# kspalaiologos/bzip3

Hardware: AMD Instinct MI355X
Metric: MiB/s encode+decode round-trip, 8 MiB blocks (higher is better)
Workload: dtype u8

## Files before the change

### bzip3_amd/__init__.py

```python
import ctypes as C
import os

_HERE = os.path.dirname(os.path.abspath(__file__))
LIB_PATH = os.path.join(_HERE, "lib", "libbzip3.so")

BZ3_OK = 0
BZ3_ERR_OUT_OF_BOUNDS = -1
BZ3_ERR_BWT = -2
BZ3_ERR_CRC = -3
BZ3_ERR_MALFORMED_HEADER = -4
BZ3_ERR_TRUNCATED_DATA = -5
BZ3_ERR_DATA_TOO_BIG = -6
BZ3_ERR_INIT = -7
BZ3_ERR_DATA_SIZE_TOO_SMALL = -8

T_NAMES = ["crc", "rle", "lzp", "bwt", "cm", "copy", "_6", "_7"]

_lib = None


def _declare(L, strict=True):
    vp, i32, u32, sz = C.c_void_p, C.c_int32, C.c_uint32, C.c_size_t
    sig = {
        "bz3_version": (C.c_char_p, []),
        "bz3_last_error": (C.c_int8, [vp]),
        "bz3_strerror": (C.c_char_p, [vp]),
        "bz3_new": (vp, [i32]),
        "bz3_free": (None, [vp]),
        "bz3_bound": (sz, [sz]),
        "bz3_compress": (C.c_int, [u32, vp, vp, sz, C.POINTER(sz)]),
        "bz3_decompress": (C.c_int, [vp, vp, sz, C.POINTER(sz)]),
        "bz3_min_memory_needed": (sz, [i32]),
        "bz3_encode_block": (i32, [vp, vp, i32]),
        "bz3_decode_block": (i32, [vp, vp, sz, i32, i32]),
        "bz3_encode_blocks": (None, [vp, vp, vp, i32]),
        "bz3_decode_blocks": (None, [vp, vp, vp, vp, vp, i32]),
        "bz3_orig_size_sufficient_for_decode": (C.c_int, [vp, sz, i32]),
        "bz3_hip_device_count": (C.c_int, []),
        "bz3_hip_bind_device": (C.c_int, [C.c_int]),
        "bz3_hip_state_device": (C.c_int, [vp]),
        "bz3_hip_set_cm_mode": (C.c_int, [C.c_int]),
        "bz3_hip_cm_blocks_given_up": (C.c_uint, []),
        "bz3_hip_cm_blocks_routed_full": (C.c_uint, []),
        "bz3_hip_debug_bwt_big_rounds": (None, [C.c_int]),
        "bz3_hip_debug_peak_concurrent_groups": (C.c_int, [C.c_int]),
        "bz3_hip_debug_front_end_ring": (C.c_int, []),
        "bz3_hip_debug_arena_swap_buffers": (C.c_int, [C.c_int]),
        "bz3_hip_cm_variant_for": (C.c_int, [C.c_int, C.c_int, C.c_int]),
        "bz3_hip_set_lean_states": (C.c_int, [C.c_int]),
        "bz3_hip_release_cached_memory": (None, []),
        "bz3_hip_set_keep_workspace": (C.c_int, [C.c_int]),
        "bz3_hip_set_front_end_duo": (C.c_int, [C.c_int]),
        "bz3_hip_set_workspace_headroom": (None, [C.c_longlong]),
        "bz3_hip_workspace_headroom": (sz, []),
        "bz3_hip_debug_headroom_events": (C.c_uint, [C.c_int, C.POINTER(C.c_uint)]),
        "bz3_hip_debug_ring_contexts": (sz, [sz, sz, sz, sz, sz, sz, C.c_int, sz]),
        "bz3_hip_debug_arena_slack": (sz, [sz]),
        "bz3_hip_debug_cm_launches": (C.c_uint, [C.c_int]),
        "bz3_hip_debug_workspace_bytes": (sz, [sz, C.c_int]),
        "bz3_hip_debug_cached_bytes": (sz, [C.c_int]),
        "bz3_hip_encode_block_device": (i32, [vp, vp, i32]),
        "bz3_hip_decode_block_device": (i32, [vp, vp, sz, i32, i32]),
        "bz3_hip_encode_blocks_device": (None, [vp, vp, vp, i32]),
        "bz3_hip_decode_blocks_device": (None, [vp, vp, vp, vp, vp, i32]),
        "bz3_hip_compress_device": (C.c_int, [u32, vp, vp, sz, C.POINTER(sz)]),
        "bz3_hip_decompress_device": (C.c_int, [vp, vp, sz, C.POINTER(sz)]),
        "bz3_hip_frame_decoded_size_device": (C.c_int, [vp, sz, C.POINTER(sz)]),
        "bz3_hip_compress_device_many": (C.c_int, [u32, i32, C.POINTER(vp), C.POINTER(sz), C.POINTER(vp), C.POINTER(sz), C.POINTER(C.c_int)]),
        "bz3_hip_decompress_device_many": (C.c_int, [i32, C.POINTER(vp), C.POINTER(sz), C.POINTER(vp), C.POINTER(sz), C.POINTER(C.c_int)]),
        "bz3_hip_frame_decoded_sizes_device": (C.c_int, [i32, C.POINTER(vp), C.POINTER(sz), C.POINTER(sz), C.POINTER(C.c_int)]),
        "bz3_hip_debug_copy_segments": (i32, [vp, vp, C.POINTER(C.c_uint64), i32]),
        "bz3_hip_compress_device_planes": (C.c_int, [u32, u32, vp, vp, sz, C.POINTER(sz)]),
        "bz3_hip_decompress_device_planes": (C.c_int, [u32, vp, vp, sz, C.POINTER(sz)]),
        "bz3_hip_compress_device_planes_many": (C.c_int, [u32, i32, C.POINTER(u32), C.POINTER(vp), C.POINTER(sz), C.POINTER(vp), C.POINTER(sz), C.POINTER(C.c_int)]),
        "bz3_hip_decompress_device_planes_many": (C.c_int, [i32, C.POINTER(u32), C.POINTER(vp), C.POINTER(sz), C.POINTER(vp), C.POINTER(sz), C.POINTER(C.c_int)]),
        "bz3_hip_debug_planes": (i32, [vp, vp, C.POINTER(C.c_uint64), i32]),
        "bz3_hip_compress_device_delta": (C.c_int, [u32, u32, vp, vp, vp, sz, C.POINTER(sz)]),
        "bz3_hip_decompress_device_delta": (C.c_int, [u32, vp, vp, sz, vp, sz, C.POINTER(sz)]),
        "bz3_hip_compress_device_delta_many": (C.c_int, [u32, i32, C.POINTER(u32), C.POINTER(vp), C.POINTER(vp), C.POINTER(sz), C.POINTER(vp), C.POINTER(sz), C.POINTER(C.c_int)]),
        "bz3_hip_decompress_device_delta_many": (C.c_int, [i32, C.POINTER(u32), C.POINTER(vp), C.POINTER(sz), C.POINTER(vp), C.POINTER(sz), C.POINTER(vp), C.POINTER(sz), C.POINTER(C.c_int)]),
        "bz3_hip_crc32c_device": (C.c_int, [vp, sz, u32, C.POINTER(u32)]),
        "bz3_hip_debug_delta": (i32, [vp, vp, vp, C.POINTER(C.c_uint64), i32]),
        "bz3_hip_decompress_device_range": (C.c_int, [u32, vp, sz, C.c_uint64, vp, sz, vp, C.POINTER(sz)]),
        "bz3_hip_decompress_device_range_many": (C.c_int, [i32, C.POINTER(u32), C.POINTER(vp), C.POINTER(sz), C.POINTER(C.c_uint64), C.POINTER(vp), C.POINTER(sz),
                                                           C.POINTER(vp), C.POINTER(sz), C.POINTER(C.c_int)]),
# ... 705 lines not shown
```

### bzip3_amd/csrc/api.hip

```cpp
#include <atomic>
#include <chrono>
#include <condition_variable>
#include <cstdio>
#include <cstdlib>
#include <exception>
#include <mutex>
#include <new>
#include <stdexcept>
#include <thread>
#include <type_traits>
#include <vector>

#include "../../include/bz3_hip.h"
#include "frame.hpp"
#include "planes.hpp"
#include "prims.hpp"
#include "sort.hpp"
#include "stages.hpp"

using namespace bz3;

namespace {

constexpr s32 KiB65 = 65 * 1024;
// ... 79 lines not shown
#endif
            for (int k = 0; k < AUX; k++) {
                HIP_CHECK(hipStreamCreateWithFlags(&st[k], hipStreamNonBlocking));
                HIP_CHECK(hipEventCreate(&e0[k]));
                HIP_CHECK(hipEventCreate(&e1[k]));
            }
            HIP_CHECK(hipStreamCreateWithFlags(&du, hipStreamNonBlocking));
        } catch (...) {
            if (du) (void)hipStreamDestroy(du);
            if (ep) (void)hipEventDestroy(ep);
            if (rs) (void)hipStreamDestroy(rs);
            for (int k = 0; k < AUX; k++)
                if (sm[k]) (void)hipStreamDestroy(sm[k]);
            for (int k = 0; k < AUX; k++) {
                if (st[k]) (void)hipStreamDestroy(st[k]);
                if (e0[k]) (void)hipEventDestroy(e0[k]);
                if (e1[k]) (void)hipEventDestroy(e1[k]);
            }
            throw;
        }
        ev_prep = ep;
        duo = du;
        rest = rs;
        for (int k = 0; k < AUX; k++) aux_m[k] = sm[k];
        reserved_cus = reserved;
        for (int k = 0; k < AUX; k++) {
            aux[k] = st[k];
            ev_d0[k] = e0[k];
            ev_d1[k] = e1[k];
        }
        aux_ready = true;
    }

    std::mutex temp_mu;
    std::vector<std::pair<u8 *, size_t>> temps_free;
    std::vector<std::pair<u8 *, size_t>> temps_out;
    u8 * temp_get(size_t cap) {
        std::lock_guard<std::mutex> lk(temp_mu);
        for (size_t k = 0; k < temps_free.size(); k++)
            if (temps_free[k].second >= cap) {
                auto t = temps_free[k];
                temps_free.erase(temps_free.begin() + (long)k);
                temps_out.push_back(t);
                return t.first;
            }
        u8 * p = nullptr;
        if (hipMalloc((void **)&p, cap) != hipSuccess) {
            (void)hipGetLastError();
            (void)hipDeviceSynchronize();
            for (auto & t : temps_free) (void)hipFree(t.first);
            temps_free.clear();
            HIP_CHECK(hipMalloc((void **)&p, cap));
        }
        temps_out.push_back({p, cap});
        return p;
    }
    void temp_put(u8 * p) {
        if (!p) return;
        std::lock_guard<std::mutex> lk(temp_mu);
        for (size_t k = 0; k < temps_out.size(); k++)
            if (temps_out[k].first == p) {
                temps_free.push_back(temps_out[k]);
                temps_out.erase(temps_out.begin() + (long)k);
                return;
            }
    }
// ... 368 lines not shown
    if (total <= base || !ctx_bytes) return 0;
    size_t by_share = (total - base) / 10 * 7 / ctx_bytes;
    const size_t aside = headroom + ((size_t)513 << 20) + ((size_t)64 << 20);
    const size_t room = total > base + aside ? total - base - aside : 0;
    if (!lean) {
        const size_t by_room = room / ctx_bytes;
        return by_share < by_room ? by_share : by_room;
    }
    return room / (ctx_bytes + cap);
}
void enforce_headroom(DeviceCtx * ctx, hipStream_t s);

#ifndef BZ3_FRONT_DUO_DEFAULT
#define BZ3_FRONT_DUO_DEFAULT 0
#endif
std::atomic<int> g_keep_ws{-1};
inline bool keep_workspace() {
    static const bool env_on = [] {
        const char * e = getenv("BZ3_HIP_KEEP_WS");
        return e && atoi(e) != 0;
    }();
    const int v = g_keep_ws.load();
    return v < 0 ? env_on : v != 0;
}
std::atomic<int> g_front_duo{-1};
inline bool front_end_duo() {
    static const int env_on = [] {
        const char * e = getenv("BZ3_HIP_FRONT_DUO");
        return e ? (atoi(e) != 0 ? 1 : 0) : BZ3_FRONT_DUO_DEFAULT;
    }();
    const int v = g_front_duo.load();
    return v < 0 ? env_on != 0 : v != 0;
}
inline void lean_borrow(bz3_state * st) {
    if (st->lean && !st->d_swap) st->d_swap = st->ctx->temp_get(st->cap);
}
inline void lean_return(bz3_state * st) {
    if (st->lean && st->d_swap) {
        st->ctx->temp_put(st->d_swap);
        st->d_swap = nullptr;
    }
}
constexpr u32 CM_SIDE_BYTES = 64 * 1024;

void encode_front_a(bz3_state * st, u8 * buf, s32 data_size, Arena & arena, Arena & ctx_arena, LzpEncodeCtx & c) {
    st->pending = bz3_state::FAILED;
    st->result = -1;
    c.active = false;
    if (st->skip) return;
    if (data_size > st->block_size || data_size < 0) {
        st->last_error = BZ3_ERR_DATA_TOO_BIG;
        return;
    }
    hipStream_t s = st->xs;
    for (float & x : st->t) x = 0.f;
    double t0 = now_ms();
    crc32c_device(buf, (u64)data_size, 1u, st->ctx->d_crc, st->d_words, s);
    st->user = buf;
    st->size = data_size;
    if (data_size < 64) {
        launch(k_store_small, dim3(1), dim3(64), 0, s, buf, (u32)data_size, (const u32 *)(st->d_words + 1));
        st->pending = bz3_state::ENC_STORED;
        return;
    }
    if (st->timed) {
        HIP_CHECK(hipStreamSynchronize(s));
// ... 143 lines not shown
    if (const char * e = getenv("BZ3_HIP_LZP_PIPE")) {
        int w = 0, q = 0;
        if (sscanf(e, "%d,%d", &w, &q) == 2 && w >= 1 && q >= 2 && q <= DeviceCtx::AUX) {
            window = w;
            ns = q;
        }
    }
    if (window > n) window = n;
    if (window < 1) window = 1;
}

void encode_group(bz3_state ** sts, u8 ** bufs, const s32 * sizes, s32 n) {
    if (n <= 0) return;
    bz3_state * lead = sts[0];
    DeviceGuard g(lead->device);
    std::lock_guard<std::mutex> lk(lead->ctx->mu);
    for (s32 i = 0; i < n; i++) {
        sts[i]->xs = lead->stream;
        sts[i]->timed = i == 0;
    }
    size_t need = 0, need_a = 0, need_b = 0;
    for (s32 i = 0; i < n; i++) {
        const u64 nb = (u64)(sizes[i] > 0 ? sizes[i] : 0) + 64;
        const size_t w = workspace_bytes_for(nb), wa = front_a_scratch_bytes(nb), wb = front_b_scratch_bytes(nb);
        if (w > need) need = w;
        if (wa > need_a) need_a = wa;
        if (wb > need_b) need_b = wb;
    }
    const bool duo_wanted = front_end_duo() && n >= 16;
    if (duo_wanted) need = need_a + need_b + 65536;
    u64 n_max = 64;
    for (s32 i = 0; i < n; i++)
        if (sizes[i] > 0 && (u64)sizes[i] > n_max) n_max = (u64)sizes[i];
    const size_t ctx_bytes = lzp_encode_ctx_bytes(n_max + 64) + 65536;
    const size_t headroom = ws_headroom();
    const size_t fixed = (size_t)n * (sizeof(CmEncodeJob) + CM_SIDE_BYTES + 256) + cm_scratch_bytes((size_t)n) + 65536 + (size_t)DeviceCtx::AUX * 8 * (sizeof(LzpDriverJob) + 256);
    size_t contexts = ((size_t)32 << 30) / ctx_bytes;
    {
        size_t free_b = 0, total_b = 0;
        const s32 full = DeviceCtx::RING_SLOTS * 8;
        if (lead->lean && lead->ctx->temp_idle_bytes() > 0 && hipMemGetInfo(&free_b, &total_b) == hipSuccess) {
            if (ring_contexts_for(free_b, lead->ctx->ws_cap, need, fixed, ctx_bytes, lead->cap, true, headroom) < (size_t)(n < full ? n : full)) lead->ctx->temp_trim();
        }
        if (hipMemGetInfo(&free_b, &total_b) == hipSuccess)
            contexts = ring_contexts_for(free_b, lead->ctx->ws_cap, need, fixed, ctx_bytes, lead->cap, lead->lean, headroom);
    }
    s32 window = 1, ns = 2;
    pipeline_shape((s32)(contexts < 1024 ? contexts : 1024), n, window, ns);
    lead->ctx->ensure_aux();
    hipStream_t s = lead->stream;
    DrainOnUnwind drain{s, lead->ctx->aux, DeviceCtx::AUX};
    static const bool front_rest = [] { const char * e = getenv("BZ3_HIP_FRONT_REST"); return e && atoi(e) != 0; }();
    if (front_rest && lead->ctx->rest && n > 1) {
        s = lead->ctx->rest;
        for (s32 i = 0; i < n; i++) sts[i]->xs = s;
    }
    DrainOnUnwind drain_rest{s == lead->stream ? nullptr : s, nullptr, 0};
    Arena arena;
    for (;;) {
        try {
            arena = lead->ctx->arena_for(need + (size_t)ns * (size_t)window * (ctx_bytes + sizeof(LzpDriverJob) + 256) +
                                         (size_t)n * (sizeof(CmEncodeJob) + CM_SIDE_BYTES + 256) + cm_scratch_bytes((size_t)n) + 65536);
            break;
        } catch (const HipError &) {
            if (ns == 2 && window == 1) throw;
            (void)hipGetLastError();
            if (ns > 2) ns = 2;
            else window = (window + 1) / 2;
        }
    }
    g_front_end_ring.store(window | (ns << 16));
    CmEncodeJob * d_jobs = arena.take<CmEncodeJob>((size_t)n);
    u8 * sides = arena.take<u8>((size_t)n * CM_SIDE_BYTES);
    struct Window {
        s32 w0 = 0, w1 = 0;
        Arena slot;
        LzpDriverJob * d_lz = nullptr;
        std::vector<LzpEncodeCtx> ctxs;
        std::vector<LzpDriverJob> lz;
    } win[DeviceCtx::AUX];
    for (int k = 0; k < ns; k++) {
        win[k].slot.base = arena.take<char>((size_t)window * ctx_bytes);
        win[k].slot.cap = (size_t)window * ctx_bytes;
        win[k].d_lz = arena.take<LzpDriverJob>((size_t)window);
    }
    std::vector<CmEncodeJob> jobs;
    std::vector<s32> job_owner;
    const s32 nwin = (n + window - 1) / window;
    const s32 lag = ns - 1;
    static const bool trace_rings = getenv("BZ3_HIP_TRACE_RINGS") != nullptr;
    double tr_prep = 0, tr_wait = 0, tr_fin = 0, tr_t0 = now_ms();
    auto prepare = [&](s32 k, hipStream_t sp, Arena & scr, hipEvent_t ev) {
        const int q = (int)(k % ns);
        Window & w = win[q];
        w.w0 = k * window;
        w.w1 = (w.w0 + window < n) ? w.w0 + window : n;
        w.slot.used = 0;
        w.ctxs.assign((size_t)(w.w1 - w.w0), LzpEncodeCtx());
        w.lz.clear();
        for (s32 i = w.w0; i < w.w1; i++) {
            sts[i]->xs = sp;
            sts[i]->hold_swap = false;
            encode_front_a(sts[i], bufs[i], sizes[i], scr, w.slot, w.ctxs[(size_t)(i - w.w0)]);
            if (sts[i]->pending == bz3_state::ENC_CODED && w.ctxs[(size_t)(i - w.w0)].active) w.lz.push_back(lzp_driver_job(w.ctxs[(size_t)(i - w.w0)]));
        }
        HIP_CHECK(hipEventRecord(ev, sp));
        if (!w.lz.empty()) {
            hipStream_t sq = lead->ctx->aux[q];
            HIP_CHECK(hipStreamWaitEvent(sq, ev, 0));
            HIP_CHECK(hipEventRecord(lead->ctx->ev_d0[q], sq));
            lzp_driver_batch(w.lz.data(), w.d_lz, (u32)w.lz.size(), sq);
            HIP_CHECK(hipEventRecord(lead->ctx->ev_d1[q], sq));
        }
    };
    auto finish = [&](s32 j, hipStream_t sf, Arena & scr, std::vector<bz3_state *> * held) {
        const int q = (int)(j % ns);
        Window & w = win[q];
        float driver_ms = 0.f;
        if (!w.lz.empty()) {
            const double t0 = now_ms();
            HIP_CHECK(hipEventSynchronize(lead->ctx->ev_d1[q]));
            (void)hipEventElapsedTime(&driver_ms, lead->ctx->ev_d0[q], lead->ctx->ev_d1[q]);
            tr_wait += now_ms() - t0;
        }
        for (s32 i = w.w0; i < w.w1; i++) {
            sts[i]->xs = sf;
            sts[i]->hold_swap = held != nullptr;
            encode_front_b(sts[i], scr, w.ctxs[(size_t)(i - w.w0)], driver_ms);
            sts[i]->hold_swap = false;
            if (sts[i]->pending == bz3_state::ENC_CODED) {
                CmEncodeJob j2{dev_addr(sts[i]->b2), dev_addr(sts[i]->b1 + sts[i]->overhead * 4 + 1), dev_addr(sts[i]->d_words + 2), sts[i]->n_cm, 0u};
                if (sts[i]->lean) {
                    sts[i]->side = sides + (size_t)i * CM_SIDE_BYTES;
                    j2.gap = (u32)(sts[i]->b2 - (sts[i]->b1 + sts[i]->overhead * 4 + 1));
                    j2.side = dev_addr(sts[i]->side);
                    j2.side_cap = CM_SIDE_BYTES;
                }
                jobs.push_back(j2);
                job_owner.push_back(i);
            }
            if (held) {
                if (sts[i]->lean && sts[i]->d_swap) held->push_back(sts[i]);
            } else {
                lean_return(sts[i]);
            }
        }
    };
    const bool duo = duo_wanted && nwin >= 3 && lead->ctx->aux_ready && s == lead->stream;
    if (!duo) {
        for (s32 k = 0; k < nwin + lag; k++) {
            const double tr_a = now_ms();
            if (k < nwin) prepare(k, s, arena, lead->ctx->ev_prep);
            const double tr_b = now_ms();
            tr_prep += tr_b - tr_a;
            if (k >= lag) finish(k - lag, s, arena, nullptr);
            tr_fin += now_ms() - tr_b;
        }
    } else {
        g_front_end_ring.fetch_or(1 << 29);
        hipStream_t sA = lead->ctx->duo;
        DrainOnUnwind drain_duo{sA, nullptr, 0};
        Arena scr_a;
        scr_a.base = arena.take<char>(need_a);
        scr_a.cap = need_a;
        struct Events {
            std::vector<hipEvent_t> e;
            ~Events() {
                for (hipEvent_t x : e)
                    if (x) (void)hipEventDestroy(x);
            }
        } evs;
        evs.e.assign((size_t)2 * (size_t)nwin, nullptr);
        for (auto & x : evs.e) HIP_CHECK(hipEventCreateWithFlags(&x, hipEventDisableTiming));
        hipEvent_t * evA = evs.e.data(), * evB = evs.e.data() + nwin;
        struct Shared {
            std::mutex m;
            std::condition_variable cv;
            s32 prepared = 0, finished = 0;
            bool abort = false;
            std::exception_ptr err;
            std::mutex pool;
            hipEvent_t last_return = nullptr;
// ... 52 lines not shown
            }
        } joiner{ta, sh};
        std::vector<bz3_state *> held;
        for (s32 j = 0; j < nwin; j++) {
            const double tr_b = now_ms();
            {
                std::unique_lock<std::mutex> ul(sh.m);
                sh.cv.wait(ul, [&] { return sh.abort || sh.prepared >= j + 1; });
                if (sh.abort) break;
            }
            HIP_CHECK(hipStreamWaitEvent(s, evA[j], 0));
            held.clear();
            finish(j, s, arena, &held);
            HIP_CHECK(hipEventRecord(evB[j], s));
            {
                std::lock_guard<std::mutex> pl(sh.pool);
                for (bz3_state * st : held) lean_return(st);
                sh.last_return = evB[j];
            }
            {
                std::lock_guard<std::mutex> ul(sh.m);
                sh.finished = j + 1;
            }
            sh.cv.notify_all();
            tr_fin += now_ms() - tr_b;
        }
        ta.join();
        if (sh.err) std::rethrow_exception(sh.err);
        HIP_CHECK(hipStreamSynchronize(sA));
        tr_prep = sh.prep_ms;
        for (s32 i = 0; i < n; i++) sts[i]->xs = s;
    }
    if (trace_rings)
        fprintf(stderr, "[bz3 rings] encode front end: %d blocks, %d windows of %d x %d slots: %.1f ms = CRC / mRLE / LZP prepare %.1f + waiting for a window's LZP drivers %.1f + LZP emit / BWT / header %.1f\n",
                (int)n, (int)nwin, (int)window, (int)ns, now_ms() - tr_t0, tr_prep, tr_wait, tr_fin - tr_wait);
    if (s != lead->stream) {
        HIP_CHECK(hipStreamSynchronize(s));
        s = lead->stream;
        for (s32 i = 0; i < n; i++) sts[i]->xs = s;
    }
    std::vector<char> to_full(jobs.size(), 0);
    if (jobs.size() > (size_t)lead->ctx->cus) {
        std::vector<u32> outside(jobs.size(), 0u);
        for (size_t k = 0; k < jobs.size(); k++) HIP_CHECK(hipMemcpyAsync(&outside[k], sts[job_owner[k]]->d_words + 8, 4, hipMemcpyDeviceToHost, lead->stream));
        HIP_CHECK(hipStreamSynchronize(lead->stream));
        for (size_t k = 0; k < jobs.size(); k++) to_full[k] = outside[k] > jobs[k].n / 4u ? 1 : 0;
    }
    const float cm_ms = run_cm_jobs(lead->ctx, arena, jobs, d_jobs, lead->stream, lead->ev0, lead->ev1,
                                    [](const CmEncodeJob * j, u32 nj, hipStream_t st, int variant) { cm_encode_batch(j, nj, st, variant); }, &to_full);
    for (s32 i = 0; i < n; i++) encode_finish(sts[i], cm_ms);
    size_t slack = (size_t)16 << 30;
    if (const char * e = getenv("BZ3_HIP_WS_KEEP_MB")) slack = (size_t)strtoull(e, nullptr, 10) << 20;
    if (lead->ctx->ws_cap > 2 * need + slack && !(keep_workspace() && lead->lean)) {
        HIP_CHECK(hipStreamSynchronize(s));
        (void)hipFree(lead->ctx->ws);
        lead->ctx->ws = nullptr;
        lead->ctx->ws_cap = 0;
        g_front_end_ring.fetch_or(1 << 30);
    }
    enforce_headroom(lead->ctx, lead->stream);
}

void decode_front(bz3_state * st, u8 * buf, size_t buffer_size, s32 compressed_size, s32 orig_size, const u8 * hdr) {
    st->pending = bz3_state::FAILED;
    st->result = -1;
    if (st->skip) return;
    if (buffer_size < 9 || buffer_size < (size_t)compressed_size) {
        st->last_error = BZ3_ERR_DATA_SIZE_TOO_SMALL;
// ... 717 lines not shown
}

BZIP3_API unsigned bz3_hip_cm_blocks_routed_full(void) { return g_cm_routed_full.load(); }
BZIP3_API void bz3_hip_set_workspace_headroom(long long bytes) { g_ws_headroom.store(bytes < 0 ? -1 : bytes); }
BZIP3_API size_t bz3_hip_workspace_headroom(void) { return ws_headroom(); }
BZIP3_API unsigned bz3_hip_debug_headroom_events(int reset, unsigned * releases) {
    const unsigned t = reset ? g_headroom_trims.exchange(0) : g_headroom_trims.load();
    const unsigned r = reset ? g_headroom_releases.exchange(0) : g_headroom_releases.load();
    if (releases) *releases = r;
    return t;
}
BZIP3_API size_t bz3_hip_debug_ring_contexts(size_t free_b, size_t have, size_t need, size_t fixed, size_t ctx_bytes, size_t cap, int lean, size_t headroom) {
    return ring_contexts_for(free_b, have, need, fixed, ctx_bytes, cap, lean != 0, headroom);
}
BZIP3_API size_t bz3_hip_debug_workspace_bytes(size_t block_bytes, int which) {
    return which == 0 ? workspace_bytes_for((u64)block_bytes + 64) : lzp_encode_ctx_bytes((u64)block_bytes + 64) + 65536;
}
BZIP3_API unsigned bz3_hip_debug_cm_launches(int reset) { return reset ? g_cm_launches.exchange(0) : g_cm_launches.load(); }
BZIP3_API size_t bz3_hip_debug_arena_slack(size_t bytes) { return DeviceCtx::arena_slack(bytes); }
BZIP3_API size_t bz3_hip_debug_cached_bytes(int device) {
    DeviceCtx * c = nullptr;
    {
        std::lock_guard<std::mutex> lk(g_mu);
        if (device >= 0 && (size_t)device < g_ctx.size()) c = g_ctx[(size_t)device];
    }
    if (!c) return 0;
    std::lock_guard<std::mutex> lk(c->mu);
    return c->ws_cap + c->temp_idle_bytes();
}
BZIP3_API int bz3_hip_set_front_end_duo(int on) {
    g_front_duo.store(on < 0 ? -1 : (on ? 1 : 0));
    return 0;
}
BZIP3_API int bz3_hip_set_keep_workspace(int on) {
    g_keep_ws.store(on < 0 ? -1 : (on ? 1 : 0));
    return 0;
}
BZIP3_API void bz3_hip_set_collect_window_us(int us) { g_collect_window_us.store(us < 0 ? 200 : us); }
BZIP3_API unsigned bz3_hip_debug_collected_batches(int reset, unsigned * largest) {
    if (largest) *largest = g_collect_largest.load();
    const unsigned b = g_collect_batches.load();
    if (reset) {
        g_collect_batches.store(0);
        g_collect_largest.store(0);
    }
    return b;
}

BZIP3_API int32_t bz3_encode_block(struct bz3_state * st, uint8_t * buffer, int32_t size) {
    SingleReq r{st, buffer, 0, size, 0};
    try {
        collect(0, r);
    } catch (...) {
        on_failure(st);
        return -1;
    }
    return r.size;
}

BZIP3_API int32_t bz3_decode_block(struct bz3_state * st, uint8_t * buffer, size_t buffer_size, int32_t compressed_size, int32_t orig_size) {
    SingleReq r{st, buffer, buffer_size, compressed_size, orig_size};
    try {
        collect(1, r);
    } catch (...) {
        on_failure(st);
        return -1;
// ... 1528 lines not shown
```

### bzip3_amd/csrc/bwt.hip

```cpp
#include <atomic>
#include <vector>

#include "prims.hpp"
#include "sort.hpp"
#include "stages.hpp"

namespace bz3 {

constexpr int BW_BLOCK = 256;
constexpr u32 V_HEAD = 0x80000000u;
constexpr u32 V_MASK = 0x3FFFFFFFu;

__global__ void __launch_bounds__(256) k_bwt_outside(const u32 * __restrict__ hist, u32 keep, u32 * __restrict__ out) {
    __shared__ u32 h[256];
    __shared__ u32 red[256 / WAVE + 1];
    const u32 c = threadIdx.x;
    h[c] = hist[c];
    __syncthreads();
    const u32 mine = h[c];
    u32 rank = 0;
    for (u32 k = 0; k < 256u; k++) rank += (h[k] > mine || (h[k] == mine && k < c)) ? 1u : 0u;
    const u32 tot = block_sum<256>(rank >= keep ? mine : 0u, red);
    if (c == 0) *out = tot;
}
// ... 1291 lines not shown
        radix_pass<K>(kk[cur], kk[cur ^ 1], (const u32 *)vv[cur], vv[cur ^ 1], n, shift, 0xFFFFFFFFu, 0u, tmp, s);
        cur ^= 1;
        st.radix_passes++;
    }
    return cur;
}

struct BwtSwitches {
    bool trace;
    int big_rounds_default;
    std::atomic<int> big_rounds;
};
static BwtSwitches & bwt_switches() {
    static BwtSwitches sw{getenv("BZ3_BWT_TRACE") != nullptr, getenv("BZ3_BWT_BIG_ROUNDS") ? atoi(getenv("BZ3_BWT_BIG_ROUNDS")) : 1,
                          {getenv("BZ3_BWT_BIG_ROUNDS") ? atoi(getenv("BZ3_BWT_BIG_ROUNDS")) : 1}};
    return sw;
}
void bwt_set_big_rounds(int k) { bwt_switches().big_rounds.store(k < 0 ? bwt_switches().big_rounds_default : k); }
struct BwtGrids {
    u32 wide, tail;
};
static BwtGrids bwt_grids(u32 n) {
    static const BwtGrids forced = [] {
        BwtGrids g{0, 0};
        if (const char * e = getenv("BZ3_BWT_GRIDS")) (void)sscanf(e, "%u,%u", &g.wide, &g.tail);
        return g;
    }();
    if (forced.wide && forced.tail) return forced;
    const u32 tail = n / (64u * 4u), wide = n / (64u * 4u * 16u);
    return BwtGrids{wide < 8u ? 8u : wide, tail < 32u ? 32u : tail};
}

__global__ void k_bwt_set_word(u32 * p, u32 v) { *p = v; }

s32 bwt_forward(const u8 * d_in, u32 n, u8 * d_out, Arena & tmp, hipStream_t s, BwtStats * stats, u32 * d_idx, u32 * d_outside) {
    if (d_outside && n < 2) HIP_CHECK(hipMemsetAsync(d_outside, 0, 4, s));
    if (n == 0) {
        if (d_idx) launch(k_bwt_set_word, dim3(1), dim3(1), 0, s, d_idx, 0u);
        return 0;
    }
    if (n == 1) {
        HIP_CHECK(hipMemcpyAsync(d_out, d_in, 1, hipMemcpyDeviceToDevice, s));
        if (d_idx) {
            launch(k_bwt_set_word, dim3(1), dim3(1), 0, s, d_idx, 1u);
            return 0;
        }
        HIP_CHECK(hipStreamSynchronize(s));
        return 1;
    }
    if (n > V_MASK) throw HipError{hipErrorUnknown, "block too large for the suffix sorter", __FILE__, __LINE__};
    const size_t mk = tmp.mark();
    u64 * key[2] = {tmp.take<u64>(n), tmp.take<u64>(n)};
    u32 * val[2] = {tmp.take<u32>(n), tmp.take<u32>(n)};
    u8 * pb = tmp.take<u8>(n);
    const u32 tiles = (u32)(((u64)n + TR_S - 1) / TR_S);
    u32 * tile_last = tmp.take<u32>(tiles + 1);
    u32 * carry = tmp.take<u32>(tiles + 1);
    const u32 sp_groups = (tiles + SP_GROUP - 1) / SP_GROUP;
    u32 * group_max = tmp.take<u32>(sp_groups + 1);
    u32 * group_carry = tmp.take<u32>(sp_groups + 1);
    u8 * dirty = tmp.take<u8>(tiles + 2);
    u32 * hbits = tmp.take<u32>(((size_t)n + 63) / 64 * 2 + (size_t)TR_S / 32 + 8);
    u32 * d_words = tmp.take<u32>(16);
    u32 * d_vlc = tmp.take<u32>(256);
    u32 * d_hist = tmp.take<u32>(256);
    BwtStats st;

    auto grid = [](u64 m) { return dim3((u32)((m + BW_BLOCK - 1) / BW_BLOCK)); };

    HIP_CHECK(hipMemsetAsync(d_hist, 0, 256 * sizeof(u32), s));
    HIP_CHECK(hipMemsetAsync(d_words, 0, 16 * sizeof(u32), s));
    HIP_CHECK(hipMemsetAsync(d_words + 5, 0xFF, sizeof(u32), s));
    launch(k_bwt_sym_hist, grid(((u64)n + 63) / 64), dim3(BW_BLOCK), 0, s, d_in, n, d_hist);
    if (d_outside) launch(k_bwt_outside, dim3(1), dim3(256), 0, s, (const u32 *)d_hist, (u32)BWT_ROUTE_KEEP, d_outside);
    {
        const size_t vm = tmp.mark();
        vlc_build_device(d_hist, d_vlc, tmp, s);
        tmp.release(vm);
    }

    launch(k_bwt_vlc_keys, grid(((u64)n + 7) / 8), dim3(BW_BLOCK), 0, s, d_in, n, (const u32 *)d_vlc, key[0]);
    const int cur = sort_iota<u64>(key[0], key[0], key[1], val[0], val[1], n, 8, 64, tmp, s, st);
    st.sorted_elements += n;
    st.rounds++;
    u32 * V = val[cur];
    launch(k_bwt_heads, dim3(tiles), dim3(BW_BLOCK), 0, s, (const u64 *)key[cur], V, pb, n, tile_last, hbits, d_words);
    launch(k_bwt_spine_a, dim3(sp_groups), dim3(SP_BLOCK), 0, s, (const u32 *)tile_last, tiles, carry, group_max);
    launch(k_bwt_spine_b, dim3(1), dim3(1024), 0, s, (const u32 *)group_max, sp_groups, group_carry);

    const u32 big_cap = n / 4;
    char * scratch = reinterpret_cast<char *>(key[0]);
    (void)scratch;
    u32 * big_slot = reinterpret_cast<u32 *>(key[0]);
    u32 * big_hp = big_slot + big_cap;
    u32 * bord[2] = {big_hp + big_cap, big_hp + 2 * (size_t)big_cap};
    u32 * bgk[2] = {bord[1] + big_cap, bord[1] + 2 * (size_t)big_cap};
    u32 * gv = bgk[1] + big_cap;
    u32 * ghp = gv + big_cap;
    u64 * bkey0 = key[1];
    u64 * bkey[2] = {bkey0 + big_cap, bkey0 + 2 * (size_t)big_cap};
    u64 * gkey = bkey0 + 3 * (size_t)big_cap;
    u8 * gpb = reinterpret_cast<u8 *>(val[cur ^ 1]);
    const u32 tail_cap = n;
    u32 * tail_v = tmp.take<u32>(tail_cap);
    u32 * tail_slot = tmp.take<u32>(tail_cap);
// ... 25 lines not shown
        const int max_big = bwt_switches().big_rounds.load();
        if (h_words[3] || pass >= max_big || nb > n / 4) {
            deep = true;
            break;
        }
        st.rounds++;
        st.sorted_elements += nb;
        launch(k_big_keys, grid(nb), dim3(BW_BLOCK), 0, s, d_in, n, (const u32 *)V, (const u32 *)d_vlc, (const u32 *)big_slot, nb, (u32)pass + 1u, bkey0);
        int c = sort_iota<u64>(bkey0, bkey[0], bkey[1], bord[0], bord[1], nb, 0, 57, tmp, s, st);
        u32 * order = bord[c];
        u32 * ofree = bord[c ^ 1];
        launch(k_big_order_keys, grid(nb), dim3(BW_BLOCK), 0, s, (const u32 *)order, (const u32 *)big_hp, nb, bgk[0]);
        {
            const int hb = bits_for(n);
            u32 * oo[2] = {order, ofree};
            const int c2 = radix_sort_pairs<u32>(bgk[0], bgk[1], oo[0], oo[1], nb, 0, hb, tmp, s);
            st.radix_passes += (hb + 7) / 8;
            order = oo[c2];
            ofree = oo[c2 ^ 1];
        }
        launch(k_big_gather, grid(nb), dim3(BW_BLOCK), 0, s, (const u32 *)order, (const u32 *)big_slot, (const u32 *)big_hp, (const u64 *)bkey0, (const u32 *)V,
               (const u8 *)pb, nb, gv, gpb, gkey, ghp);
        {
            const int hb = bits_for(n);
            HIP_CHECK(hipMemcpyAsync(bgk[0], big_slot, (size_t)nb * 4, hipMemcpyDeviceToDevice, s));
            u32 * oo[2] = {order, ofree};
            const int c3 = radix_sort_pairs<u32>(bgk[0], bgk[1], oo[0], oo[1], nb, 0, hb, tmp, s);
            st.radix_passes += (hb + 7) / 8;
            HIP_CHECK(hipMemsetAsync(dirty, 0, tiles + 2, s));
            launch(k_big_apply, grid(nb), dim3(BW_BLOCK), 0, s, (const u32 *)bgk[c3], (const u32 *)gv, (const u8 *)gpb, (const u64 *)gkey, (const u32 *)ghp, nb, V, pb,
                   dirty, d_words);
        }
        g += 7;
        HIP_CHECK(hipMemsetAsync(d_words, 0, sizeof(u32), s));
        HIP_CHECK(hipMemsetAsync(d_words + 4, 0, sizeof(u32), s));
        HIP_CHECK(hipMemsetAsync(d_words + 5, 0xFF, sizeof(u32), s));
        HIP_CHECK(hipMemsetAsync(d_words + 8, 0, sizeof(u32), s));
        launch(k_bwt_reduce_heads, dim3(tiles), dim3(BW_BLOCK), 0, s, (const u32 *)V, n, tile_last, hbits);
        launch(k_bwt_spine_a, dim3(sp_groups), dim3(SP_BLOCK), 0, s, (const u32 *)tile_last, tiles, carry, group_max);
    launch(k_bwt_spine_b, dim3(1), dim3(1024), 0, s, (const u32 *)group_max, sp_groups, group_carry);
    }

    u32 idx = 0;
    if (!deep) {
        launch(k_bwt_finish, grid(n), dim3(BW_BLOCK), 0, s, d_in, (const u8 *)pb, n, (const u32 *)(d_words + 2), d_out, d_words + 7);
    } else {
        u32 * sa = V;
        u32 * isa = tmp.take<u32>(n);
        u32 * slot[2] = {tmp.take<u32>(n), tmp.take<u32>(n)};
        u32 * grp = tmp.take<u32>(n);
        u32 * vv[2] = {val[cur ^ 1], tmp.take<u32>(n)};
        const u32 max_tiles = (u32)(((u64)n + BG_TILE - 1) / BG_TILE);
        u32 * tile_head = tmp.take<u32>(2 * (size_t)max_tiles + 16);
        u32 * tile_keep = tile_head + max_tiles + 8;
        u32 m = n, h = g < 7u + 5u * (u32)TL_CAP ? g : 7u + 5u * (u32)TL_CAP;
        if (bwt_switches().trace) fprintf(stderr, "[bwt] n %u deep path from depth %u\n", n, h);
        {
            u32 * rk = reinterpret_cast<u32 *>(key[0]);
            u32 * kb = rk + n;
            u32 * rb = reinterpret_cast<u32 *>(key[1]);
            const u32 tl = (u32)(((u64)m + BG_TILE - 1) / BG_TILE);
            launch(k_bg_reduce<true>, dim3(tl), dim3(BW_BLOCK), 0, s, (const u64 *)nullptr, (const u32 *)V, m, tile_head, tile_keep);
            launch(k_bg_spine, dim3(1), dim3(BG_SPINE), 0, s, tile_head, tile_keep, tl, d_words + 6);
            launch(k_bg_apply<true, false>, dim3(tl), dim3(BW_BLOCK), 0, s, (const u64 *)nullptr, (const u32 *)V, (const u32 *)nullptr, m, (const u32 *)tile_head,
                   (const u32 *)tile_keep, sa, isa, vv[0], slot[0], grp, d_in, pb, rk);
            const int nbits = bits_for((u64)n - 1);
            const int shift = nbits > 8 ? nbits - 8 : 0;
            radix_pass<u32>((const u32 *)V, kb, (const u32 *)rk, rb, n, shift, 0xFFFFFFFFu, 0u, tmp, s);
            st.radix_passes++;
            const u32 itiles = (u32)(((u64)n + BW_BLOCK * IS_ITEMS - 1) / (BW_BLOCK * IS_ITEMS));
// ... 48 lines not shown
```

### include/bz3_hip.h

```cpp
#ifndef BZ3_HIP_H
#define BZ3_HIP_H
#include <stddef.h>
#include <stdint.h>
#include "libbz3.h"
#define BZ3_HIP 1

#ifdef __cplusplus
extern "C" {
#endif

BZIP3_API int bz3_hip_device_count(void);
BZIP3_API int bz3_hip_bind_device(int device);
BZIP3_API int bz3_hip_state_device(struct bz3_state * state);

BZIP3_API int bz3_hip_set_cm_mode(int mode);
BZIP3_API void bz3_hip_debug_bwt_big_rounds(int k);
BZIP3_API unsigned bz3_hip_cm_blocks_given_up(void);
BZIP3_API unsigned bz3_hip_cm_blocks_routed_full(void);

BZIP3_API int bz3_hip_cm_variant_for(int device, int blocks, int encode);

BZIP3_API int bz3_hip_debug_peak_concurrent_groups(int reset);

BZIP3_API int bz3_hip_debug_front_end_ring(void);
BZIP3_API int bz3_hip_set_keep_workspace(int on);
BZIP3_API int bz3_hip_set_front_end_duo(int on);
BZIP3_API void bz3_hip_set_workspace_headroom(long long bytes);
BZIP3_API size_t bz3_hip_workspace_headroom(void);
BZIP3_API unsigned bz3_hip_debug_headroom_events(int reset, unsigned * releases);
BZIP3_API size_t bz3_hip_debug_ring_contexts(size_t free_bytes, size_t have, size_t need, size_t fixed, size_t ctx_bytes, size_t cap, int lean, size_t headroom);
BZIP3_API size_t bz3_hip_debug_arena_slack(size_t bytes);
BZIP3_API unsigned bz3_hip_debug_cm_launches(int reset);
BZIP3_API size_t bz3_hip_debug_workspace_bytes(size_t block_bytes, int which);
BZIP3_API size_t bz3_hip_debug_cached_bytes(int device);
BZIP3_API int bz3_hip_debug_arena_swap_buffers(int reset);

BZIP3_API int bz3_hip_set_lean_states(int on);
BZIP3_API void bz3_hip_release_cached_memory(void);

BZIP3_API int32_t bz3_hip_encode_block_device(struct bz3_state * state, void * buffer, int32_t size);
BZIP3_API int32_t bz3_hip_decode_block_device(struct bz3_state * state, void * buffer, size_t buffer_size, int32_t compressed_size,
                                              int32_t orig_size);
BZIP3_API void bz3_hip_encode_blocks_device(struct bz3_state * states[], void * buffers[], int32_t sizes[], int32_t n);
BZIP3_API void bz3_hip_decode_blocks_device(struct bz3_state * states[], void * buffers[], size_t buffer_sizes[], int32_t sizes[],
                                            int32_t orig_sizes[], int32_t n);

BZIP3_API int bz3_hip_compress_device(uint32_t block_size, const void * in, void * out, size_t in_size, size_t * out_size);
BZIP3_API int bz3_hip_decompress_device(const void * in, void * out, size_t in_size, size_t * out_size);
BZIP3_API int bz3_hip_frame_decoded_size_device(const void * in, size_t in_size, size_t * decoded_size);
BZIP3_API int bz3_hip_compress_device_many(uint32_t block_size, int32_t n, const void * const ins[], const size_t in_sizes[],
                                           void * const outs[], size_t out_sizes[], int rcs[]);
BZIP3_API int bz3_hip_decompress_device_many(int32_t n, const void * const ins[], const size_t in_sizes[],
                                             void * const outs[], size_t out_sizes[], int rcs[]);
BZIP3_API int bz3_hip_frame_decoded_sizes_device(int32_t n, const void * const ins[], const size_t in_sizes[],
                                                 size_t decoded_sizes[], int rcs[]);
BZIP3_API int32_t bz3_hip_debug_copy_segments(const void * src, void * dst, const uint64_t * segs, int32_t n);

BZIP3_API int bz3_hip_compress_device_planes(uint32_t block_size, uint32_t elem_size, const void * in, void * out, size_t in_size,
                                             size_t * out_size);
// ... 69 lines not shown
```

Before: 636.1.

## Add multi-lane host threads for encode front end and fuse BWT memsets into kernels

Adds an optional multi-lane mode in which helper host threads, each with its own stream and scratch arena, run the per-block LZP emit/BWT/header stage of a window in parallel, synchronised through events. The default lane count is 1, so this path stays off unless it is enabled by env var or API. The BWT forward pass also replaces several small hipMemsetAsync calls with single tiny reset kernels, aiming to cut per-call launch overhead. The lane mode adds threading complexity and extra workspace when enabled.

```diff
diff --git a/bzip3_amd/__init__.py b/bzip3_amd/__init__.py
--- a/bzip3_amd/__init__.py
+++ b/bzip3_amd/__init__.py
@@ -51,6 +51,7 @@
         "bz3_hip_release_cached_memory": (None, []),
         "bz3_hip_set_keep_workspace": (C.c_int, [C.c_int]),
         "bz3_hip_set_front_end_duo": (C.c_int, [C.c_int]),
+        "bz3_hip_set_front_end_lanes": (C.c_int, [C.c_int]),
         "bz3_hip_set_workspace_headroom": (None, [C.c_longlong]),
         "bz3_hip_workspace_headroom": (sz, []),
         "bz3_hip_debug_headroom_events": (C.c_uint, [C.c_int, C.POINTER(C.c_uint)]),
diff --git a/bzip3_amd/csrc/api.hip b/bzip3_amd/csrc/api.hip
--- a/bzip3_amd/csrc/api.hip
+++ b/bzip3_amd/csrc/api.hip
@@ -135,6 +135,37 @@
         aux_ready = true;
     }
 
+    static constexpr int LANES = 3;
+    hipStream_t lane[LANES] = {};
+    hipEvent_t ev_lane[LANES] = {}, ev_win[AUX] = {};
+    bool lanes_ready = false;
+    void ensure_lanes() {
+        if (lanes_ready) return;
+        hipStream_t st[LANES] = {};
+        hipEvent_t el[LANES] = {}, ew[AUX] = {};
+        try {
+            for (int k = 0; k < LANES; k++) {
+                HIP_CHECK(hipStreamCreateWithFlags(&st[k], hipStreamNonBlocking));
+                HIP_CHECK(hipEventCreateWithFlags(&el[k], hipEventDisableTiming));
+            }
+            for (int k = 0; k < AUX; k++) HIP_CHECK(hipEventCreateWithFlags(&ew[k], hipEventDisableTiming));
+        } catch (...) {
+            for (int k = 0; k < LANES; k++) {
+                if (st[k]) (void)hipStreamDestroy(st[k]);
+                if (el[k]) (void)hipEventDestroy(el[k]);
+            }
+            for (int k = 0; k < AUX; k++)
+                if (ew[k]) (void)hipEventDestroy(ew[k]);
+            throw;
+        }
+        for (int k = 0; k < LANES; k++) {
+            lane[k] = st[k];
+            ev_lane[k] = el[k];
+        }
+        for (int k = 0; k < AUX; k++) ev_win[k] = ew[k];
+        lanes_ready = true;
+    }
+
     std::mutex temp_mu;
     std::vector<std::pair<u8 *, size_t>> temps_free;
     std::vector<std::pair<u8 *, size_t>> temps_out;
@@ -569,6 +600,21 @@
     const int v = g_front_duo.load();
     return v < 0 ? env_on != 0 : v != 0;
 }
+constexpr int FRONT_LANES_MAX = 4;
+constexpr u64 FRONT_LANES_BELOW = (u64)64 << 20;
+constexpr int FRONT_LANES_DEFAULT = 1;
+std::atomic<int> g_front_lanes{-1};
+inline int front_end_lanes(u64 n_max, s32 n, bool duo) {
+    static const int env = [] {
+        const char * e = getenv("BZ3_HIP_FRONT_LANES");
+        return e && *e ? atoi(e) : -1;
+    }();
+    if (duo) return 1;
+    int v = g_front_lanes.load();
+    if (v < 0) v = env;
+    if (v >= 1) return v < FRONT_LANES_MAX ? v : FRONT_LANES_MAX;
+    return n >= 8 && n_max < FRONT_LANES_BELOW ? FRONT_LANES_DEFAULT : 1;
+}
 inline void lean_borrow(bz3_state * st) {
     if (st->lean && !st->d_swap) st->d_swap = st->ctx->temp_get(st->cap);
 }
@@ -778,6 +824,9 @@
     u64 n_max = 64;
     for (s32 i = 0; i < n; i++)
         if (sizes[i] > 0 && (u64)sizes[i] > n_max) n_max = (u64)sizes[i];
+    const int lanes = n < 2 ? 1 : front_end_lanes(n_max, n, duo_wanted);
+    const size_t lane_bytes = need_b + 65536;
+    if (lanes > 1) need += (size_t)(lanes - 1) * lane_bytes;
     const size_t ctx_bytes = lzp_encode_ctx_bytes(n_max + 64) + 65536;
     const size_t headroom = ws_headroom();
     const size_t fixed = (size_t)n * (sizeof(CmEncodeJob) + CM_SIDE_BYTES + 256) + cm_scratch_bytes((size_t)n) + 65536 + (size_t)DeviceCtx::AUX * 8 * (sizeof(LzpDriverJob) + 256);
@@ -797,7 +846,7 @@
     hipStream_t s = lead->stream;
     DrainOnUnwind drain{s, lead->ctx->aux, DeviceCtx::AUX};
     static const bool front_rest = [] { const char * e = getenv("BZ3_HIP_FRONT_REST"); return e && atoi(e) != 0; }();
-    if (front_rest && lead->ctx->rest && n > 1) {
+    if (front_rest && lead->ctx->rest && n > 1 && lanes == 1) {
         s = lead->ctx->rest;
         for (s32 i = 0; i < n; i++) sts[i]->xs = s;
     }
@@ -815,7 +864,7 @@
             else window = (window + 1) / 2;
         }
     }
-    g_front_end_ring.store(window | (ns << 16));
+    g_front_end_ring.store(window | (ns << 16) | (lanes << 24));
     CmEncodeJob * d_jobs = arena.take<CmEncodeJob>((size_t)n);
     u8 * sides = arena.take<u8>((size_t)n * CM_SIDE_BYTES);
     struct Window {
@@ -859,41 +908,184 @@
             HIP_CHECK(hipEventRecord(lead->ctx->ev_d1[q], sq));
         }
     };
+    auto front_b = [&](Window & w, s32 i, hipStream_t sf, Arena & scr, float driver_ms, bool hold) {
+        sts[i]->xs = sf;
+        sts[i]->hold_swap = hold;
+        encode_front_b(sts[i], scr, w.ctxs[(size_t)(i - w.w0)], driver_ms);
+        sts[i]->hold_swap = false;
+    };
+    auto collect = [&](s32 i, std::vector<bz3_state *> * held) {
+        if (sts[i]->pending == bz3_state::ENC_CODED) {
+            CmEncodeJob j2{dev_addr(sts[i]->b2), dev_addr(sts[i]->b1 + sts[i]->overhead * 4 + 1), dev_addr(sts[i]->d_words + 2), sts[i]->n_cm, 0u};
+            if (sts[i]->lean) {
+                sts[i]->side = sides + (size_t)i * CM_SIDE_BYTES;
+                j2.gap = (u32)(sts[i]->b2 - (sts[i]->b1 + sts[i]->overhead * 4 + 1));
+                j2.side = dev_addr(sts[i]->side);
+                j2.side_cap = CM_SIDE_BYTES;
+            }
+            jobs.push_back(j2);
+            job_owner.push_back(i);
+        }
+        if (held) {
+            if (sts[i]->lean && sts[i]->d_swap) held->push_back(sts[i]);
+        } else {
+            lean_return(sts[i]);
+        }
+    };
+    auto drivers_done = [&](int q) {
+        float driver_ms = 0.f;
+        if (!win[q].lz.empty()) {
+            HIP_CHECK(hipEventSynchronize(lead->ctx->ev_d1[q]));
+            (void)hipEventElapsedTime(&driver_ms, lead->ctx->ev_d0[q], lead->ctx->ev_d1[q]);
+        }
+        return driver_ms;
+    };
     auto finish = [&](s32 j, hipStream_t sf, Arena & scr, std::vector<bz3_state *> * held) {
         const int q = (int)(j % ns);
         Window & w = win[q];
-        float driver_ms = 0.f;
-        if (!w.lz.empty()) {
-            const double t0 = now_ms();
-            HIP_CHECK(hipEventSynchronize(lead->ctx->ev_d1[q]));
-            (void)hipEventElapsedTime(&driver_ms, lead->ctx->ev_d0[q], lead->ctx->ev_d1[q]);
-            tr_wait += now_ms() - t0;
-        }
+        const double t0 = now_ms();
+        const float driver_ms = drivers_done(q);
+        tr_wait += now_ms() - t0;
         for (s32 i = w.w0; i < w.w1; i++) {
-            sts[i]->xs = sf;
-            sts[i]->hold_swap = held != nullptr;
-            encode_front_b(sts[i], scr, w.ctxs[(size_t)(i - w.w0)], driver_ms);
-            sts[i]->hold_swap = false;
-            if (sts[i]->pending == bz3_state::ENC_CODED) {
-                CmEncodeJob j2{dev_addr(sts[i]->b2), dev_addr(sts[i]->b1 + sts[i]->overhead * 4 + 1), dev_addr(sts[i]->d_words + 2), sts[i]->n_cm, 0u};
-                if (sts[i]->lean) {
-                    sts[i]->side = sides + (size_t)i * CM_SIDE_BYTES;
-                    j2.gap = (u32)(sts[i]->b2 - (sts[i]->b1 + sts[i]->overhead * 4 + 1));
-                    j2.side = dev_addr(sts[i]->side);
-                    j2.side_cap = CM_SIDE_BYTES;
-                }
-                jobs.push_back(j2);
-                job_owner.push_back(i);
-            }
-            if (held) {
-                if (sts[i]->lean && sts[i]->d_swap) held->push_back(sts[i]);
-            } else {
-                lean_return(sts[i]);
-            }
+            front_b(w, i, sf, scr, driver_ms, held != nullptr);
+            collect(i, held);
         }
     };
     const bool duo = duo_wanted && nwin >= 3 && lead->ctx->aux_ready && s == lead->stream;
-    if (!duo) {
+    if (lanes > 1) {
+        DeviceCtx * const ctx = lead->ctx;
+        ctx->ensure_lanes();
+        DrainOnUnwind drain_lanes{nullptr, ctx->lane, DeviceCtx::LANES};
+        Arena scr_lane[DeviceCtx::LANES];
+        for (int l = 0; l + 1 < lanes; l++) {
+            scr_lane[l].base = arena.take<char>(lane_bytes);
+            scr_lane[l].cap = lane_bytes;
+        }
+        struct Shared {
+            std::mutex m;
+            std::condition_variable cv;
+            s32 gen = 0;
+            int q = 0;
+            s32 next = 0, end = 0;
+            int busy = 0;
+            bool touched[DeviceCtx::LANES] = {};
+            bool quit = false;
+            std::exception_ptr err;
+        } sh;
+        const int device = lead->device;
+        auto helper = [&](int l) {
+            s32 seen = 0;
+            for (;;) {
+                int q = 0;
+                {
+                    std::unique_lock<std::mutex> ul(sh.m);
+                    sh.cv.wait(ul, [&] { return sh.quit || sh.gen != seen; });
+                    if (sh.quit) return;
+                    seen = sh.gen;
+                    if (sh.next >= sh.end) continue;
+                    q = sh.q;
+                    sh.busy++;
+                }
+                bool ran = false;
+                try {
+                    Window & w = win[q];
+                    float driver_ms = 0.f;
+                    for (;;) {
+                        s32 i;
+                        {
+                            std::lock_guard<std::mutex> ul(sh.m);
+                            if (sh.quit || sh.next >= sh.end) break;
+                            i = sh.next++;
+                        }
+                        if (!ran) {
+                            driver_ms = drivers_done(q);
+                            HIP_CHECK(hipStreamWaitEvent(ctx->lane[l], ctx->ev_win[q], 0));
+                            ran = true;
+                        }
+                        front_b(w, i, ctx->lane[l], scr_lane[l], driver_ms, true);
+                    }
+                    if (ran) HIP_CHECK(hipEventRecord(ctx->ev_lane[l], ctx->lane[l]));
+                } catch (...) {
+                    std::lock_guard<std::mutex> ul(sh.m);
+                    if (!sh.err) sh.err = std::current_exception();
+                    sh.quit = true;
+                }
+                {
+                    std::lock_guard<std::mutex> ul(sh.m);
+                    sh.busy--;
+                    if (ran) sh.touched[l] = true;
+                }
+                sh.cv.notify_all();
+            }
+        };
+        std::thread th[DeviceCtx::LANES];
+        struct Joiner {
+            std::thread * t;
+            Shared & sh;
+            ~Joiner() {
+                {
+                    std::lock_guard<std::mutex> ul(sh.m);
+                    sh.quit = true;
+                }
+                sh.cv.notify_all();
+                for (int l = 0; l < DeviceCtx::LANES; l++)
+                    if (t[l].joinable()) t[l].join();
+            }
+        } joiner{th, sh};
+        for (int l = 0; l + 1 < lanes; l++)
+            th[l] = std::thread([&helper, l, device] {
+                (void)hipSetDevice(device);
+                helper(l);
+            });
+        for (s32 k = 0; k < nwin + lag; k++) {
+            const double tr_a = now_ms();
+            const s32 j = k - lag;
+            const int q = j >= 0 ? (int)(j % ns) : 0;
+            if (j >= 0) {
+                std::lock_guard<std::mutex> ul(sh.m);
+                sh.q = q;
+                sh.next = win[q].w0;
+                sh.end = win[q].w1;
+                sh.gen++;
+            }
+            if (j >= 0) sh.cv.notify_all();
+            if (k < nwin) prepare(k, s, arena, ctx->ev_win[k % ns]);
+            const double tr_b = now_ms();
+            tr_prep += tr_b - tr_a;
+            if (j < 0) continue;
+            Window & w = win[q];
+            float driver_ms = 0.f;
+            bool ran = false;
+            for (;;) {
+                s32 i;
+                {
+                    std::lock_guard<std::mutex> ul(sh.m);
+                    if (sh.quit || sh.next >= sh.end) break;
+                    i = sh.next++;
+                }
+                if (!ran) {
+                    const double t0 = now_ms();
+                    driver_ms = drivers_done(q);
+                    tr_wait += now_ms() - t0;
+                    ran = true;
+                }
+                front_b(w, i, s, arena, driver_ms, true);
+            }
+            {
+                std::unique_lock<std::mutex> ul(sh.m);
+                sh.cv.wait(ul, [&] { return sh.busy == 0; });
+                if (sh.err) std::rethrow_exception(sh.err);
+                for (int l = 0; l + 1 < lanes; l++)
+                    if (sh.touched[l]) {
+                        HIP_CHECK(hipStreamWaitEvent(s, ctx->ev_lane[l], 0));
+                        sh.touched[l] = false;
+                    }
+            }
+            for (s32 i = w.w0; i < w.w1; i++) collect(i, nullptr);
+            tr_fin += now_ms() - tr_b;
+        }
+        for (s32 i = 0; i < n; i++) sts[i]->xs = s;
+    } else if (!duo) {
         for (s32 k = 0; k < nwin + lag; k++) {
             const double tr_a = now_ms();
             if (k < nwin) prepare(k, s, arena, lead->ctx->ev_prep);
@@ -1012,8 +1204,8 @@
         for (s32 i = 0; i < n; i++) sts[i]->xs = s;
     }
     if (trace_rings)
-        fprintf(stderr, "[bz3 rings] encode front end: %d blocks, %d windows of %d x %d slots: %.1f ms = CRC / mRLE / LZP prepare %.1f + waiting for a window's LZP drivers %.1f + LZP emit / BWT / header %.1f\n",
-                (int)n, (int)nwin, (int)window, (int)ns, now_ms() - tr_t0, tr_prep, tr_wait, tr_fin - tr_wait);
+        fprintf(stderr, "[bz3 rings] encode front end: %d blocks, %d windows of %d x %d slots, %d lane(s): %.1f ms = CRC / mRLE / LZP prepare %.1f + waiting for a window's LZP drivers %.1f + LZP emit / BWT / header %.1f\n",
+                (int)n, (int)nwin, (int)window, (int)ns, lanes, now_ms() - tr_t0, tr_prep, tr_wait, tr_fin - tr_wait);
     if (s != lead->stream) {
         HIP_CHECK(hipStreamSynchronize(s));
         s = lead->stream;
@@ -1797,6 +1989,11 @@
     g_front_duo.store(on < 0 ? -1 : (on ? 1 : 0));
     return 0;
 }
+BZIP3_API int bz3_hip_set_front_end_lanes(int lanes) {
+    if (lanes == 0 || lanes > FRONT_LANES_MAX) return -1;
+    g_front_lanes.store(lanes < 0 ? -1 : lanes);
+    return 0;
+}
 BZIP3_API int bz3_hip_set_keep_workspace(int on) {
     g_keep_ws.store(on < 0 ? -1 : (on ? 1 : 0));
     return 0;
diff --git a/bzip3_amd/csrc/bwt.hip b/bzip3_amd/csrc/bwt.hip
--- a/bzip3_amd/csrc/bwt.hip
+++ b/bzip3_amd/csrc/bwt.hip
@@ -1347,6 +1347,16 @@
 }
 
 __global__ void k_bwt_set_word(u32 * p, u32 v) { *p = v; }
+__global__ void k_bwt_reset_all(u32 * hist, u32 * w) {
+    const u32 t = threadIdx.x;
+    hist[t] = 0u;
+    if (t < 16u) w[t] = t == 5u ? 0xFFFFFFFFu : 0u;
+}
+__global__ void k_bwt_reset_pass(u32 * w) {
+    const u32 t = threadIdx.x;
+    if (t == 0u || t == 4u || t == 8u) w[t] = 0u;
+    if (t == 5u) w[t] = 0xFFFFFFFFu;
+}
 
 s32 bwt_forward(const u8 * d_in, u32 n, u8 * d_out, Arena & tmp, hipStream_t s, BwtStats * stats, u32 * d_idx, u32 * d_outside) {
     if (d_outside && n < 2) HIP_CHECK(hipMemsetAsync(d_outside, 0, 4, s));
@@ -1383,9 +1393,7 @@
 
     auto grid = [](u64 m) { return dim3((u32)((m + BW_BLOCK - 1) / BW_BLOCK)); };
 
-    HIP_CHECK(hipMemsetAsync(d_hist, 0, 256 * sizeof(u32), s));
-    HIP_CHECK(hipMemsetAsync(d_words, 0, 16 * sizeof(u32), s));
-    HIP_CHECK(hipMemsetAsync(d_words + 5, 0xFF, sizeof(u32), s));
+    launch(k_bwt_reset_all, dim3(1), dim3(256), 0, s, d_hist, d_words);
     launch(k_bwt_sym_hist, grid(((u64)n + 63) / 64), dim3(BW_BLOCK), 0, s, d_in, n, d_hist);
     if (d_outside) launch(k_bwt_outside, dim3(1), dim3(256), 0, s, (const u32 *)d_hist, (u32)BWT_ROUTE_KEEP, d_outside);
     {
@@ -1477,10 +1485,7 @@
                    dirty, d_words);
         }
         g += 7;
-        HIP_CHECK(hipMemsetAsync(d_words, 0, sizeof(u32), s));
-        HIP_CHECK(hipMemsetAsync(d_words + 4, 0, sizeof(u32), s));
-        HIP_CHECK(hipMemsetAsync(d_words + 5, 0xFF, sizeof(u32), s));
-        HIP_CHECK(hipMemsetAsync(d_words + 8, 0, sizeof(u32), s));
+        launch(k_bwt_reset_pass, dim3(1), dim3(16), 0, s, d_words);
         launch(k_bwt_reduce_heads, dim3(tiles), dim3(BW_BLOCK), 0, s, (const u32 *)V, n, tile_last, hbits);
         launch(k_bwt_spine_a, dim3(sp_groups), dim3(SP_BLOCK), 0, s, (const u32 *)tile_last, tiles, carry, group_max);
     launch(k_bwt_spine_b, dim3(1), dim3(1024), 0, s, (const u32 *)group_max, sp_groups, group_carry);
diff --git a/include/bz3_hip.h b/include/bz3_hip.h
--- a/include/bz3_hip.h
+++ b/include/bz3_hip.h
@@ -25,6 +25,7 @@
 BZIP3_API int bz3_hip_debug_front_end_ring(void);
 BZIP3_API int bz3_hip_set_keep_workspace(int on);
 BZIP3_API int bz3_hip_set_front_end_duo(int on);
+BZIP3_API int bz3_hip_set_front_end_lanes(int lanes);
 BZIP3_API void bz3_hip_set_workspace_headroom(long long bytes);
 BZIP3_API size_t bz3_hip_workspace_headroom(void);
 BZIP3_API unsigned bz3_hip_debug_headroom_events(int reset, unsigned * releases);
```

Result: no change. 634.8 (-0.2%).
